# zhouzypaul/fql

Hardware: AMD Instinct MI355X
Metric: FQL gradient-steps/s (batch=256) (higher is better)
Workload: dtype f32

## Files before the change

fql_amd/csrc/fql_engine.hip:

```cpp
#include "../../include/fql_amd.h"
#include "fql_kernels.h"
#include "fql_conv.h"
#include "fql_chain.h"
#include "fql_aux.h"
#include "fql_ifql.h"
#include "fql_rebrac.h"
#include "fql_sac.h"
#include "fql_bc.h"
#include "fql_iql.h"
#include "fql_iqld.h"
#include "fql_cfgrl.h"
#include <hip/hip_ext.h>
#include "fql_aql.h"

#include <algorithm>
#include <cmath>
#include <cstdarg>
#include <cstdio>
#include <cstdlib>
#include <cstring>
#include <map>
#include <memory>
#include <random>
#include <string>
// ... 198 lines not shown
    std::vector<WgradTask> h_wgrad;
    std::vector<LnBwdTask> h_ln;
    std::vector<MiscTask> h_misc;
    bool ka = false;
    std::vector<int> waits;
    bool record_after = false;
    hipEvent_t ev = nullptr;
};

inline bool ka_tasks_env() {
    const char* e = getenv("FQL_KERNARG_TASKS");
    return !e || atoi(e) != 0;
}
inline bool fused_tail_env() {
    const char* e = getenv("FQL_FUSED_TAIL");
    return !e || atoi(e) != 0;
}
inline bool aql_acquire_env() {
    const char* e = getenv("FQL_AQL_ACQUIRE");
    return e && atoi(e) != 0;
}
inline bool l1_independent_kernel(const void* fn) {
#define FQL_L1_CHAIN(HH)                                                                                                                             \
    (const void*)fql_chain_kernel<HH, 0>, (const void*)fql_chain_kernel<HH, 1>, (const void*)fql_chain_kernel<HH, 2>, (const void*)fql_chain_kernel<HH, 3>, \
    (const void*)fql_chain_multi_kernel<HH, 0>, (const void*)fql_chain_multi_kernel<HH, 1>, (const void*)fql_chain_multi_kernel<HH, 2>,             \
    (const void*)fql_chain_multi_kernel<HH, 3>, (const void*)fql_chain_split_kernel<HH, 0>, (const void*)fql_chain_split_kernel<HH, 1>,             \
    (const void*)fql_chain_split_kernel<HH, 2>
    static const void* const table[] = {
        (const void*)fql_prep_kernel, (const void*)fql_prep_multi_kernel,
        (const void*)fql_gemm16_kernel<false>, (const void*)fql_gemm16_kernel<true>,
// ... 312 lines not shown
    float* in_noise[5] = {nullptr, nullptr, nullptr, nullptr, nullptr};
    int64_t* in_idx = nullptr;
    float *X_os = nullptr, *X_bc = nullptr, *X_eu = nullptr, *X_c1 = nullptr, *X_c2 = nullptr, *X_ct = nullptr;
    float *vel = nullptr, *w_rew = nullptr, *w_mask = nullptr, *w_act = nullptr, *tgt = nullptr;
    float *X_e0 = nullptr, *C0 = nullptr, *Abuf[2] = {nullptr, nullptr}, *Vpart = nullptr;
    bool fused_euler = false;
    bool use_chain = false;
    int fill_lane_full = 1;
    std::vector<float*> wf_bc;
    float *wf_w0 = nullptr, *wf_w4 = nullptr;
    WfragTask* d_wfrag = nullptr;
    std::vector<WfragTask> h_wfrag;
    int wfrag_n = 0, wfrag_grid = 0;
    const bool ka_tasks = ka_tasks_env();
    const bool fused_tail = fused_tail_env();
    unsigned* d_ticket = nullptr;
    std::vector<void*> chain_allocs;
    bool split_build = false;
    bool wide_tiles = false;
    bool split_ok = false;
    int vp_tiles = 0;
    int num_cus = 0;
    PassBuf p_os, p_os_bwd, p_bc, p_eu, p_c1[2], p_c2[2], p_ct[2];
    Program prog_fwdbwd, prog_opt, prog_loss;
    Program prog_opt_split;
    Program prog_full;
    int mod_chunk0[3] = {0, 0, 0}, mod_chunkn[3] = {0, 0, 0};
    Program prog_split;
    hipGraphExec_t split_exec[4] = {nullptr, nullptr, nullptr, nullptr};
    hipGraph_t split_graph[4] = {nullptr, nullptr, nullptr, nullptr};
// ... 450 lines not shown
        HIP_CHECK(hipMemcpy(P, h.data(), n_total * sizeof(float), hipMemcpyHostToDevice));
    }

    PassBuf make_pass(std::vector<void*>& owner, int net, int M, float* x0, bool bwd, bool input_grad) {
        const Net& n = nets[net];
        PassBuf p;
        p.net = net; p.M = M; p.x0 = x0;
        const int L = n.nl() - 1;
        for (int l = 0; l < L; ++l) {
            const int H = n.layers[l].out_p;
            p.g.push_back(dalloc(owner, (size_t)M * H));
            p.z.push_back(dalloc(owner, (size_t)M * H));
            if (n.layers[l].ln) {
                p.xn.push_back(dalloc(owner, (size_t)M * H));
                p.stats.push_back(dalloc(owner, (size_t)M * 2));
                p.lnpart.push_back(dalloc(owner, (size_t)M * ((2 * ((H + 31) / 32) + 3) & ~3)));
            } else {
                p.xn.push_back(p.g.back());
                p.stats.push_back(nullptr);
                p.lnpart.push_back(nullptr);
            }
        }
        p.out = dalloc(owner, (size_t)M * n.layers[L].out_p);
        if (bwd) {
            for (int l = 0; l <= L; ++l) p.dz.push_back(dalloc(owner, (size_t)M * n.layers[l].out_p));
            for (int l = 0; l < L; ++l) p.dy.push_back(n.layers[l].ln ? dalloc(owner, (size_t)M * n.layers[l].out_p) : nullptr);
            if (input_grad) p.dx0 = dalloc(owner, (size_t)M * n.in_p());
        }
        return p;
    }

// ... 253 lines not shown

    void push(Program& pr, Op& op) {
        op.lane = emit_lane;
        pr.ops.push_back(op);
    }
    Op& emit(Program& pr, OpType type, const Bound& k, std::vector<const void*> reads, std::vector<const void*> writes) {
        Op op{};
        op.type = type;
        op.k = k;
        op.reads = std::move(reads);
        op.writes = std::move(writes);
        push(pr, op);
        return pr.ops.back();
    }

    void emit_forward(Program& pr, const PassBuf& p, bool save, int final_flags = 0, float* aux = nullptr,
                      float* aux2 = nullptr, float f0 = 0.f, float f1 = 0.f, int first_layer = 0) {
        const Net& n = nets[p.net];
        const int L = n.nl() - 1;
        for (int l = first_layer; l <= L; ++l) {
            const Layer& ly = n.layers[l];
            Op op{};
            op.type = OP_GEMM;
            GemmTask& t = op.gemm;
            const bool a_ln = l > 0 && n.layers[l - 1].ln;
            t.A = (l == 0) ? p.x0 : p.g[l - 1];
            t.lda = ly.in_p;
            t.B = P + ly.w; t.ldb = ly.out_p;
            t.bias = P + ly.b;
            t.M = p.M; t.N = ly.out_p; t.K = ly.in_p;
            t.ldc = ly.out_p;
            t.flags = GF_BIAS;
            op.reads = {t.A, t.B};
            if (a_ln) {
                t.flags |= GF_A_LN;
// ... 4 lines not shown
                    t.ln_xout = p.xn[l - 1]; t.ln_stats = p.stats[l - 1];
                    op.writes.push_back(t.ln_xout);
                    op.writes.push_back(t.ln_stats);
                }
            }
            if (l < L) {
                t.C = p.g[l];
                t.flags |= GF_GELU;
                if (save) { t.flags |= GF_SAVE_Z; t.Zout = p.z[l]; op.writes.push_back(t.Zout); }
                op.writes.push_back(t.C);
                const bool prev64 = l > 0 && want64(p.M, n.layers[l - 1].out_p, n.layers[l - 1].in_p, GF_BIAS | GF_GELU);
                if (want64(t.M, t.N, t.K, t.flags) && (!a_ln || prev64)) {
                    op.type = OP_GEMM64;
                    if (a_ln) { t.aux2 = p.lnpart[l - 1]; t.i0 = t.K / 32; op.reads.push_back(t.aux2); }
                    if (ly.ln) { t.flags |= GF_LN_PART; t.aux = p.lnpart[l]; t.i1 = t.N / 32; op.writes.push_back(t.aux); }
                }
            } else {
                t.C = p.out;
                t.flags |= final_flags;
                if (final_flags & GF_EULER) {
                    t.aux = aux; t.aux2 = aux2;
                    t.i0 = n.in_p(); t.i1 = cfg.obs_dim; t.i2 = cfg.act_dim;
                    t.f0 = f0; t.f1 = f1;
                    op.reads.push_back(aux);
                    op.writes.push_back(aux);
                    if (aux2) op.writes.push_back(aux2);
                } else {
                    op.writes.push_back(t.C);
                    if (final_flags & GF_OS_SCATTER) {
                        t.aux = aux; t.aux2 = aux2;
                        t.i0 = nets[NET_C0].in_p(); t.i1 = cfg.obs_dim; t.i2 = cfg.act_dim;
                        op.writes.push_back(aux);
                        op.writes.push_back(aux2);
                    }
                }
            }
            push(pr, op);
        }
    }

    void emit_euler_fused(Program& pr) {
        const Net& n = nets[NET_BC];
        const int nh = n.nl() - 1, fs = cfg.flow_steps;
        const int od = cfg.obs_dim, ad = cfg.act_dim, ap = pad16(ad), inp_b = n.in_p();
        const Layer& l0 = n.layers[0];
        {
            Op op{};
            op.type = OP_GEMM;
            GemmTask& t = op.gemm;
            t.A = X_e0; t.lda = l0.in_p; t.B = P + l0.w; t.ldb = l0.out_p; t.bias = P + l0.b; t.C = C0; t.ldc = l0.out_p;
            t.M = B; t.N = l0.out_p; t.K = l0.in_p; t.flags = GF_BIAS;
            op.reads = {X_e0, t.B};
            op.writes = {C0};
// ... 146 lines not shown
    }
    void emit_wfrag(Program& pr) {
        if (!use_chain) return;
        const Net& n = nets[NET_BC];
        Op op{};
        op.type = OP_WFRAG;
        op.k = tl_last(bind(fql_wfrag_kernel, wfrag_grid, d_wfrag, wfrag_n, -1));
        for (const Layer& L : n.layers) op.reads.push_back(P + L.w);
        for (float* w : wf_bc) op.writes.push_back(w);
        op.writes.push_back(wf_w0);
        op.writes.push_back(wf_w4);
        push(pr, op);
    }

    void emit_backward(Program& pr, const PassBuf& p, int row_off, int M, bool param_grads, bool input_grad,
                       const void* align_with = nullptr) {
        size_t first_op = pr.ops.size();
        const Net& n = nets[p.net];
        const int L = n.nl() - 1;
        auto rows = [&](float* base, int ld) { return base + (size_t)row_off * ld; };
        auto ln_bwd = [&](int l, const void* first_read) {
            const Layer& prev = n.layers[l - 1];
            Op lo{};
            lo.type = OP_LNBWD;
            LnBwdTask& q = lo.ln;
            q.Z = rows(p.z[l - 1], prev.out_p);
            q.Gv = rows(p.g[l - 1], prev.out_p);
            q.stats = p.stats[l - 1] + (size_t)row_off * 2;
            q.gamma = P + prev.g;
            q.dZ = p.dz[l - 1];
            q.dgamma = param_grads ? G + prev.g : nullptr;
// ... 19 lines not shown
                w.db = G + ly.b;
                w.M = M; w.Kin = ly.in_p; w.N = ly.out_p;
                op.reads = {xin_id, dz};
                op.writes = {w.dW, w.db};
                const int keep = emit_lane;
                if (emit_lane == 0 && !split_build && !lane0_64) emit_lane = 1;
                if (defer_wgrads) { op.lane = emit_lane; defer_wgrads->push_back(op); }
                else push(pr, op);
                emit_lane = keep;
            }
            if (l == 0 && !input_grad) break;
            if (l == L && l > 0 && ly.out == 1 && n.layers[l - 1].ln) {
                Op lo = ln_bwd(l, dz);
                LnBwdTask& q = lo.ln;
                q.dq = dz; q.ldq = ly.out_p; q.wq = P + ly.w; q.ldw = ly.out_p;
                push(pr, lo);
                continue;
            }
            Op op{};
            op.type = OP_GEMM;
            GemmTask& t = op.gemm;
            t.A = dz; t.lda = ly.out_p;
            t.B = P + ly.w; t.ldb = ly.out_p;
            t.M = M; t.N = ly.in_p; t.K = ly.out_p;
            t.ldc = ly.in_p;
            t.flags = GF_TRANS_B;
            op.reads = {dz, t.B};
            if (l == 0) {
                t.C = p.dx0;
                op.writes = {t.C};
// ... 349 lines not shown
            GemmTask t = o->gemm;
            t.wk = (t.N <= 16) ? 4 : 2;
            t.tmt = 1;
            t.ntn = (t.N / 16 + (4 / t.wk) - 1) / (4 / t.wk);
            t.tile0 = tile;
            tile += (t.M / 16) * t.ntn;
            L.h_gemm.push_back(t);
        }
        L.table = upload(owner, L.h_gemm.data(), L.h_gemm.size() * sizeof(GemmTask));
        L.grid = tile;
        bind_gemm16(L);
        return L;
    }

    static double op_macs(const Op& o) {
        if (o.type == OP_GEMM || o.type == OP_GEMM64 || o.type == OP_HEAD_DGRAD) return (double)o.gemm.M * o.gemm.N * o.gemm.K;
        if (o.type == OP_DGRAD0) return (double)o.gemm.M * 16.0 * o.gemm.K;
        if (o.type == OP_WGRAD) return (double)o.wgrad.M * o.wgrad.Kin * o.wgrad.N;
        if (o.type == OP_CHAIN) return o.macs;
        if (o.type == OP_CONV || o.type == OP_CONV_U8) return (double)o.conv.N * o.conv.H * o.conv.W * 9.0 * (o.conv.transposed ? o.conv.Ci : o.conv.Ci_real) * o.conv.Co;
        if (o.type == OP_CONV_WGRAD) return (double)o.cw.N * o.cw.H * o.cw.W * 9.0 * o.cw.Ci_real * o.cw.Co;
        return 0.0;
    }
    static void cross_lane_waits(Program& pr) {
        std::vector<int> need(pr.launches.size() * FQL_LANES, -1);
        for (const Op& o : pr.ops) {
            if (o.launch < 0) continue;
            for (int d : o.deps) {
                const int dl = pr.ops[d].launch;
                const int ol = pr.launches[dl].lane;
                int& nd = need[o.launch * FQL_LANES + ol];
// ... 330 lines not shown
        if (!split_build) fill_lane_full = fill_lane;
        wide_tiles = lanes3;
        place("os", 1, true);
        emit_forward(pr, p_os, with_grads, GF_OS_SCATTER, X_ct, X_c2);
        {
            Op op{};
            op.type = OP_POSTOS;
            op.postos = PostOsArgs{p_os.out, w_act, X_ct, X_c2, st, B, od, ad, inp_c, ap};
            op.reads = {p_os.out, w_act};
            op.writes = {I_MSE};
            push(pr, op);
        }
        place("c1f", fill_lane, true);
        for (int e = 0; e < 2; ++e) emit_forward(pr, p_c1[e], with_grads);
        place("ct", lanes3 ? 1 : fill_lane, true);
        for (int e = 0; e < 2; ++e) emit_forward(pr, p_ct[e], false);
        place("c1", fill_lane, true);
        {
            Op op{};
            op.type = OP_LOSS_CRITIC;
            op.lc = LossCriticArgs{p_c1[0].out, p_c1[1].out, p_ct[0].out, p_ct[1].out, w_rew, w_mask,
                                   with_grads ? p_c1[0].dz.back() : nullptr, with_grads ? p_c1[1].dz.back() : nullptr,
                                   st, B, cfg.q_agg, with_grads ? 1 : 0, cfg.discount};
            op.reads = {p_c1[0].out, p_c1[1].out, p_ct[0].out, p_ct[1].out, w_rew, w_mask};
            op.writes = {I_CR};
            if (with_grads) { op.writes.push_back(p_c1[0].dz.back()); op.writes.push_back(p_c1[1].dz.back()); }
            push(pr, op);
        }
        std::vector<Op> late_ops;
        if (!lanes3 && with_grads) defer_wgrads = &late_ops;
        if (with_grads)
            for (int e = 0; e < 2; ++e) emit_backward(pr, p_c1[e], 0, B, true, visual);
        const bool enc_align = !split_build;
        if (with_grads && visual && !enc_align) {
            place("enc", 1, true);
            emit_encoder_backward(pr, eb_c, 0, B, p_c1[0].dx0, p_c1[1].dx0, nets[NET_C0].in_p());
        }
        {
            place("bcf", lanes3 ? 1 : fill_lane, true);
// ... 4 lines not shown
                op.type = OP_LOSS_BC;
                op.lb = LossBcArgs{p_bc.out, vel, with_grads ? p_bc.dz.back() : nullptr, st, B, ad, ap, with_grads ? 1 : 0};
                op.reads = {p_bc.out, vel};
                op.writes = {I_BC};
                if (with_grads) op.writes.push_back(p_bc.dz.back());
                push(pr, op);
            }
            defer_wgrads = nullptr;
            if (with_grads) emit_backward(pr, p_bc, 0, B, true, visual);
            if (with_grads && visual && !enc_align) {
                place("enc", 1, true);
                emit_encoder_backward(pr, eb_bc, 0, B, p_bc.dx0, nullptr, nets[NET_BC].in_p());
            }
        }
        place("c2", 1, true);
        for (int e = 0; e < 2; ++e) emit_forward(pr, p_c2[e], with_grads);
        {
            Op op{};
            op.type = OP_LOSS_Q;
            const bool dyn_dq = with_grads && cfg.normalize_q_loss;
            op.lq = LossQArgs{p_c2[0].out, p_c2[1].out, dyn_dq ? p_c2[0].dz.back() : nullptr,
                              dyn_dq ? p_c2[1].dz.back() : nullptr, st, B, cfg.normalize_q_loss, dyn_dq ? 1 : 0};
            op.reads = {p_c2[0].out, p_c2[1].out};
            op.writes = {I_Q};
            if (dyn_dq) { op.writes.push_back(p_c2[0].dz.back()); op.writes.push_back(p_c2[1].dz.back()); }
            push(pr, op);
        }
        defer_wgrads = nullptr;
        if (with_grads) {
            for (int e = 0; e < 2; ++e) emit_backward(pr, p_c2[e], 0, B, false, true, !lanes3 ? I_CR : nullptr);
        }
        for (Op& w : late_ops) {
            w.reads.push_back(p_c2[0].dx0); w.reads.push_back(p_c2[1].dx0);
            emit_lane = w.lane;
            push(pr, w);
        }
        place("eu", 0, false);
        const int fs = cfg.flow_steps;
        euler_finish_fused = with_grads && !cfg.actor_layer_norm && fused_euler && use_chain && fs > 1 && vp_tiles <= 32;
        if (fused_euler && use_chain) emit_euler_chain(pr);
        else if (fused_euler) emit_euler_fused(pr);
        else
        for (int s = 0; s < fs; ++s)
            emit_forward(pr, p_eu, false, GF_EULER | (s == fs - 1 ? GF_EULER_LAST : 0), X_eu, tgt, 1.0f / (float)fs,
                         (float)(s + 1) / (float)fs);
// ... 3370 lines not shown
```

fql_amd/csrc/fql_kernels.h:

```cpp
#pragma once
#include <hip/hip_runtime.h>
#include <stdint.h>

typedef float f32x4 __attribute__((ext_vector_type(4)));

#define FQL_GAS __attribute__((address_space(1)))
__device__ __forceinline__ float ldg(const float* p) { return *(const FQL_GAS float*)p; }
__device__ __forceinline__ f32x4 ldg4(const float* p) { return *(const FQL_GAS f32x4*)p; }
typedef unsigned u32x4 __attribute__((ext_vector_type(4)));
__device__ __forceinline__ __amdgpu_buffer_rsrc_t ldx_rsrc(const void* base) {
    const uint64_t b = (uint64_t)base;
    const uint64_t u = ((uint64_t)(unsigned)__builtin_amdgcn_readfirstlane((int)(b >> 32)) << 32) | (unsigned)__builtin_amdgcn_readfirstlane((int)b);
    return __builtin_amdgcn_make_buffer_rsrc((void*)u, 0, 0x7FFFFFFF, 0x00020000);
}
__device__ __forceinline__ float ldx(const float* p) { return __hip_atomic_load((const FQL_GAS float*)p, __ATOMIC_RELAXED, __HIP_MEMORY_SCOPE_AGENT); }
__device__ __forceinline__ u32x4 ldx4u(const unsigned* base, unsigned i, unsigned s = 0) {
    return __builtin_amdgcn_raw_buffer_load_b128(ldx_rsrc(base), (int)(i * 4u), __builtin_amdgcn_readfirstlane((int)(s * 4u)), 16);
}
typedef float f32x2 __attribute__((ext_vector_type(2)));
typedef unsigned u32x2 __attribute__((ext_vector_type(2)));
__device__ __forceinline__ f32x2 ldx2(const float* base, unsigned i, unsigned s = 0) {
    return __builtin_bit_cast(f32x2, __builtin_amdgcn_raw_buffer_load_b64(ldx_rsrc(base), (int)(i * 4u), __builtin_amdgcn_readfirstlane((int)(s * 4u)), 16));
}
__device__ __forceinline__ f32x4 ldx4(const float* base, unsigned i, unsigned s = 0) { return __builtin_bit_cast(f32x4, ldx4u((const unsigned*)base, i, s)); }
// ... 82 lines not shown
    GF_LN_WRITE = 1 << 5,
    GF_GELUGRAD = 1 << 6,
    GF_EULER = 1 << 7,
    GF_EULER_LAST = 1 << 8,
    GF_CLIP_OUT = 1 << 9,
    GF_A_EULER0 = 1 << 11,
    GF_HEAD_PART = 1 << 12,
    GF_OS_SCATTER = 1 << 13,
    GF_A_LOSSACT = 1 << 17,
    GF_A_EULFIN = 1 << 15,
    GF_RELUGRAD = 1 << 14,
    GF_LN_PART = 1 << 10,
    GF_C_FRAGT = 1 << 16,
    GF_C_FRAG = 1 << 18,
    GF_EULER_BARE = 1 << 19,
};

struct GemmTask {
    const float* A;
    const float* B;
    const float* bias;
    float* C;
    float* Zout;
    const float* Zprev;
    const float* ln_g;
    const float* ln_b;
    float* ln_xout;
    float* ln_stats;
    float* aux;
    float* aux2;
// ... 683 lines not shown
        f32x4 pv[NR][4];
#pragma unroll
        for (int i = 0; i < NR; ++i) {
            const unsigned po = (unsigned)((row_first + 16 * i) * rs);
#pragma unroll
            for (int t = 0; t < 4; ++t) pv[i][t] = ldx4(partials, po + 4 * min(base + t, nf4 - 1));
        }
#pragma unroll
        for (int i = 0; i < NR; ++i)
#pragma unroll
            for (int t = 0; t < 4; ++t) {
                if (2 * (base + t) < ntin) { sum[i] += pv[i][t][0]; sumsq[i] += pv[i][t][1]; }
                if (2 * (base + t) + 1 < ntin) { sum[i] += pv[i][t][2]; sumsq[i] += pv[i][t][3]; }
            }
    }
}

template <bool transb, int RI>
__device__ __forceinline__ void gemm64_body(const GemmTask& T, float* lds) {
    constexpr int TM = 32 * RI;
    float* As = lds;
    float* Bs = lds + 2 * TM * G64_S;
    float* part = Bs + 2 * 64 * G64_S;
    const int local = (int)blockIdx.x - T.tile0;
    const int tm = sdiv(local, frcp(T.ntn)), tn = local - tm * T.ntn;
    const int row0 = tm * TM, n0 = tn * 64;
    const int K = T.K;
    const int tid = threadIdx.x, wave = tid >> 6, lane = tid & 63;
    const int wr = wave >> 1, wc = wave & 1;
    const int c = lane & 15, q = lane >> 4;
// ... 248 lines not shown
                }
                if (ln_wr) stg4(T.ln_xout + (size_t)(row0 + sr + 16 * i) * T.lda + k, ra[i]);
            }
        }
#pragma unroll
        for (int i = 0; i < 2; ++i) *reinterpret_cast<f32x4*>(a + (sr + 16 * i) * G64_S + 4 * sc4) = ra[i];
#pragma unroll
        for (int i = 0; i < NB; ++i) *reinterpret_cast<f32x4*>(b + (br0 + brs * i) * BS + 4 * bc4) = rb[i];
    };
    f32x4 acc[NJ][2];
#pragma unroll
    for (int j = 0; j < NJ; ++j) acc[j][0] = acc[j][1] = f32x4{0.f, 0.f, 0.f, 0.f};
    f32x4 bias[NJ];
#pragma unroll
    for (int j = 0; j < NJ; ++j) bias[j] = (flags & GF_BIAS) ? ldg4(T.bias + n0 + (wc * NJ + j) * 16 + 4 * q) : f32x4{0.f, 0.f, 0.f, 0.f};

    auto compute = [&](int buf) {
        const float* a = As + buf * 32 * G64_S + (16 * wr + c) * G64_S + 4 * q;
        const float* b = Bs + buf * BROWS * BS;
        f32x4 fa[2], fb[2][NJ];
        auto read_frags = [&](int slot, int g) {
            fa[slot] = *reinterpret_cast<const f32x4*>(a + 16 * g);
#pragma unroll
            for (int j = 0; j < NJ; ++j) {
                const int col = (wc * NJ + j) * 16 + c;
                if (transb) fb[slot][j] = *reinterpret_cast<const f32x4*>(b + col * BS + 16 * g + 4 * q);
                else {
#pragma unroll
                    for (int s4 = 0; s4 < 4; ++s4) fb[slot][j][s4] = b[(16 * g + 4 * q + s4) * BS + col];
                }
// ... 16 lines not shown
    TSTAMP();
    for (int ch = 0; ch < nchunks; ch += 2) {
        compute(0);
        if (ch + 1 < nchunks) store_chunk(ra1, rb1, lg1, lb1, 64 * (ch + 1), 1);
        __syncthreads();
        if (ch + 3 < nchunks) load_chunk(ra1, rb1, lg1, lb1, 64 * (ch + 3));
        if (ch + 1 < nchunks) {
            compute(1);
            if (ch + 2 < nchunks) store_chunk(ra0, rb0, lg0, lb0, 64 * (ch + 2), 0);
            __syncthreads();
            if (ch + 4 < nchunks) load_chunk(ra0, rb0, lg0, lb0, 64 * (ch + 4));
        }
    }
    TSTAMP();

    float s1 = 0.f, s2 = 0.f;
    {
        const int row = row0 + 16 * wr + c;
#pragma unroll
        for (int j = 0; j < NJ; ++j) {
            const int n = n0 + (wc * NJ + j) * 16 + 4 * q;
            const size_t o = (size_t)row * T.ldc + n;
            f32x4 v = acc[j][0] + acc[j][1] + bias[j];
            if (flags & GF_SAVE_Z) {
                f32x4 dgv;
#pragma unroll
                for (int r = 0; r < 4; ++r) { float gg, dg; gelu_both(v[r], gg, dg); dgv[r] = dg; v[r] = (flags & GF_GELU) ? gg : v[r]; }
                stg4(T.Zout + o, dgv);
            } else if (flags & GF_GELU) {
#pragma unroll
                for (int r = 0; r < 4; ++r) v[r] = gelu_f(v[r]);
            }
            if (flags & GF_GELUGRAD) v *= ldx4(T.Zprev + (size_t)row0 * T.ldc, (unsigned)((16 * wr + c) * T.ldc + n));
            if (flags & GF_RELUGRAD) {
                const f32x4 zp = ldx4(T.Zprev + (size_t)row0 * T.ldc, (unsigned)((16 * wr + c) * T.ldc + n));
#pragma unroll
                for (int r = 0; r < 4; ++r) v[r] = (zp[r] > 0.f) ? v[r] : 0.f;
            }
            stg4(T.C + o, v);
#pragma unroll
            for (int r = 0; r < 4; ++r) { s1 += v[r]; s2 += v[r] * v[r]; }
        }
    }
    if (flags & GF_LN_PART) {
        s1 += __shfl_xor(s1, 16); s2 += __shfl_xor(s2, 16);
        s1 += __shfl_xor(s1, 32); s2 += __shfl_xor(s2, 32);
        if (q == 0) {
            const int rl = 16 * wr + c;
            part[(wc * 32 + rl) * 2] = s1;
            part[(wc * 32 + rl) * 2 + 1] = s2;
        }
        __syncthreads();
        const int rs = (2 * T.i1 + 3) & ~3;
        if (NJ == 2) {
            if (tid < 64) {
                const int half = tid >> 5, rl = tid & 31;
                float* pp = T.aux + (size_t)(row0 + rl) * rs + 2 * (2 * tn + half);
                stg(pp, part[(half * 32 + rl) * 2]);
                stg(pp + 1, part[(half * 32 + rl) * 2 + 1]);
            }
        } else if (tid < 32) {
            float* pp = T.aux + (size_t)(row0 + tid) * rs + 2 * tn;
            stg(pp, part[tid * 2] + part[(32 + tid) * 2]);
            stg(pp + 1, part[tid * 2 + 1] + part[(32 + tid) * 2 + 1]);
        }
    }
#ifdef FQL_STAMPS
    TSTAMP();
    if (tid == 0 && T.stamps64) {
// ... 99 lines not shown
            else {
                const int k = br0 + brs * i;
                const int key = (NJ == 2) ? ((k >> 1) & 3) : ((k >> 2) & 1);
                w = k * RW + 8 * ((bc4 >> 2) ^ key) + 2 * (bc4 & 3);
            }
            *reinterpret_cast<u32x2*>(bh + w) = hi;
            *reinterpret_cast<u32x2*>(bh + BPL + w) = lo;
        }
    };
    f32x4 acc[NJ][2];
#pragma unroll
    for (int j = 0; j < NJ; ++j) acc[j][0] = acc[j][1] = f32x4{0.f, 0.f, 0.f, 0.f};
    f32x4 bias[NJ];
#pragma unroll
    for (int j = 0; j < NJ; ++j) bias[j] = (flags & GF_BIAS) ? ldg4(T.bias + n0 + (wc * NJ + j) * 16 + 4 * q) : f32x4{0.f, 0.f, 0.f, 0.f};

    const int a_row = (16 * wr + c) * 32, sw = (c >> 1) & 7;
    const int qq = c >> 2, p = c & 3;
    const int tr_row = 4 * q + qq;
    const int tr_key = (NJ == 2) ? ((tr_row >> 1) & 3) : ((tr_row >> 2) & 1);
    auto compute = [&](int buf) {
        const unsigned* ah = As + buf * 2 * APL;
        const unsigned* bh = Bs + buf * 2 * BPL;
#pragma unroll
        for (int kp = 0; kp < 2; ++kp) {
            const int slot = 4 * ((4 * kp + q) ^ sw);
            const u32x4 fah = *reinterpret_cast<const u32x4*>(ah + a_row + slot);
            const u32x4 fal = *reinterpret_cast<const u32x4*>(ah + APL + a_row + slot);
            u32x4 fbh[NJ], fbl[NJ];
#pragma unroll
// ... 24 lines not shown
    SSTAMP();
    for (int ch = 0; ch < nchunks; ch += 2) {
        compute(0);
        if (ch + 1 < nchunks) store_chunk(ra1, rb1, lg1, lb1, 64 * (ch + 1), 1);
        __syncthreads();
        if (ch + 3 < nchunks) load_chunk(ra1, rb1, lg1, lb1, 64 * (ch + 3));
        if (ch + 1 < nchunks) {
            compute(1);
            if (ch + 2 < nchunks) store_chunk(ra0, rb0, lg0, lb0, 64 * (ch + 2), 0);
            __syncthreads();
            if (ch + 4 < nchunks) load_chunk(ra0, rb0, lg0, lb0, 64 * (ch + 4));
        }
    }

    SSTAMP();
    float s1 = 0.f, s2 = 0.f;
    {
        const int row = row0 + 16 * wr + c;
#pragma unroll
        for (int j = 0; j < NJ; ++j) {
            const int n = n0 + (wc * NJ + j) * 16 + 4 * q;
            const size_t o = (size_t)row * T.ldc + n;
            f32x4 v = acc[j][0] + acc[j][1] + bias[j];
            if (flags & GF_SAVE_Z) {
                f32x4 dgv;
#pragma unroll
                for (int r = 0; r < 4; ++r) { float gg, dg; gelu_both(v[r], gg, dg); dgv[r] = dg; v[r] = (flags & GF_GELU) ? gg : v[r]; }
                stg4(T.Zout + o, dgv);
            } else if (flags & GF_GELU) {
#pragma unroll
                for (int r = 0; r < 4; ++r) v[r] = gelu_f(v[r]);
            }
            if (flags & GF_GELUGRAD) v *= ldx4(T.Zprev + (size_t)row0 * T.ldc, (unsigned)((16 * wr + c) * T.ldc + n));
            if (flags & GF_RELUGRAD) {
                const f32x4 zp = ldx4(T.Zprev + (size_t)row0 * T.ldc, (unsigned)((16 * wr + c) * T.ldc + n));
#pragma unroll
                for (int r = 0; r < 4; ++r) v[r] = (zp[r] > 0.f) ? v[r] : 0.f;
            }
            stg4(T.C + o, v);
#pragma unroll
            for (int r = 0; r < 4; ++r) { s1 += v[r]; s2 += v[r] * v[r]; }
        }
    }
    if (flags & GF_LN_PART) {
        s1 += __shfl_xor(s1, 16); s2 += __shfl_xor(s2, 16);
        s1 += __shfl_xor(s1, 32); s2 += __shfl_xor(s2, 32);
        if (q == 0) {
            const int rl = 16 * wr + c;
            part[(wc * 32 + rl) * 2] = s1;
            part[(wc * 32 + rl) * 2 + 1] = s2;
        }
        __syncthreads();
        const int rs = (2 * T.i1 + 3) & ~3;
        if (NJ == 2) {
            if (tid < 64) {
                const int half = tid >> 5, rl = tid & 31;
                float* pp = T.aux + (size_t)(row0 + rl) * rs + 2 * (2 * tn + half);
                stg(pp, part[(half * 32 + rl) * 2]);
                stg(pp + 1, part[(half * 32 + rl) * 2 + 1]);
            }
        } else if (tid < 32) {
            float* pp = T.aux + (size_t)(row0 + tid) * rs + 2 * tn;
            stg(pp, part[tid * 2] + part[(32 + tid) * 2]);
            stg(pp + 1, part[tid * 2 + 1] + part[(32 + tid) * 2 + 1]);
        }
    }
#ifdef FQL_STAMPS
    SSTAMP();
    if (tid == 0 && T.stamps64) {
// ... 171 lines not shown
        if (s + 8 < steps) {
            if (s + 16 < steps) load(a0, b0, s + 16);
            mma(a1, b1, s + 8);
        }
    }
    wgrad_finish<1>(T, lds, acc, bs, tk, k0, n0, ntv, true);
}

template <bool SYN>
__device__ __forceinline__ void lnbwd_body(const LnBwdTask& T, int bid, float (*red)[16][16]) {
    const int local = bid - T.tile0;
    const int wave = threadIdx.x >> 6, lane = threadIdx.x & 63;
    if (local < T.ntiles_rows) {
        const int row = local * 4 + wave;
        if (row >= T.M) return;
        const float mean = ldx(T.stats + 2 * row), rstd = ldx(T.stats + 2 * row + 1);
        const unsigned ro = (unsigned)(row * T.ld);
        const float dqr = SYN ? ldx(T.dq + (size_t)row * T.ldq) : 0.f;
        f32x4 zz[4], dd[4], gm[4], gq[4];
#pragma unroll
        for (int i = 0; i < 4; ++i) {
            const int k4 = 4 * (lane + 64 * i);
            if (k4 < T.H) {
                zz[i] = ldx4(T.Z, ro + k4);
                gq[i] = ldx4(T.Gv, ro + k4);
                gm[i] = ldg4(T.gamma + k4);
                if (SYN) {
#pragma unroll
                    for (int e = 0; e < 4; ++e) dd[i][e] = dqr * ldg(T.wq + (size_t)(k4 + e) * T.ldw);
                } else dd[i] = ldx4(T.dY, ro + k4);
            } else zz[i] = gq[i] = gm[i] = dd[i] = f32x4{0.f, 0.f, 0.f, 0.f};
        }
        f32x4 d[4], xh[4];
        float s1 = 0.f, s2 = 0.f;
#pragma unroll
        for (int i = 0; i < 4; ++i)
#pragma unroll
            for (int e = 0; e < 4; ++e) {
                const int k = 4 * (lane + 64 * i) + e;
                xh[i][e] = (gq[i][e] - mean) * rstd;
                d[i][e] = dd[i][e] * gm[i][e];
                if (k < T.width) { s1 += d[i][e]; s2 += d[i][e] * xh[i][e]; }
            }
#pragma unroll
        for (int o = 1; o < 64; o <<= 1) {
            s1 += __shfl_xor(s1, o);
            s2 += __shfl_xor(s2, o);
// ... 167 lines not shown
    for (int o = 1; o < 64; o <<= 1) v += __shfl_xor(v, o);
    __syncthreads();
    if ((threadIdx.x & 63) == 0) sh[threadIdx.x >> 6] = v;
    __syncthreads();
    return sh[0] + sh[1] + sh[2] + sh[3];
}
__device__ __forceinline__ float block_max(float v, float* sh) {
#pragma unroll
    for (int o = 1; o < 64; o <<= 1) v = fmaxf(v, __shfl_xor(v, o));
    __syncthreads();
    if ((threadIdx.x & 63) == 0) sh[threadIdx.x >> 6] = v;
    __syncthreads();
    return fmaxf(fmaxf(sh[0], sh[1]), fmaxf(sh[2], sh[3]));
}

struct PostOsArgs {
    const float* A_os;
    const float* w_act;
    float *X_ct, *X_c2;
    DevState* st;
    int B, od, ad, inp_c, ap;
};
__device__ __forceinline__ void fql_post_onestep_body(const PostOsArgs& P, float* sh) {
    float se = 0.f;
    const int n = P.B * P.ad;
    for (int e = threadIdx.x; e < n; e += FQL_THREADS) {
        const int b = sdiv(e, frcp(P.ad)), a = e - b * P.ad;
        const float d = clip1(ldx(P.A_os + (size_t)(2 * P.B + b) * P.ap + a)) - ldx(P.w_act + (size_t)b * P.ap + a);
        se += d * d;
    }
    const float tot = block_sum(se, sh);
    if (threadIdx.x == 0) P.st->info[9] = tot / (float)n;
}

struct LossCriticArgs {
    const float *q1a, *q1b, *tqa, *tqb;
    const float *w_rew, *w_mask;
    float *dq1a, *dq1b;
    DevState* st;
    int B, q_agg, want_grad;
    float discount;
};
__device__ __forceinline__ void fql_loss_critic_body(const LossCriticArgs& P, float* sh) {
    float sl = 0.f, sq = 0.f, mx = -INFINITY, mn = INFINITY;
    const float gs = 1.0f / (float)P.B;
    for (int b = threadIdx.x; b < P.B; b += FQL_THREADS) {
        const float ta = ldx(P.tqa + (size_t)b * 16), tb = ldx(P.tqb + (size_t)b * 16);
        const float nq = P.q_agg ? fminf(ta, tb) : 0.5f * (ta + tb);
        const float y = ldx(P.w_rew + b) + P.discount * ldx(P.w_mask + b) * nq;
        const float qa = ldx(P.q1a + (size_t)b * 16), qb = ldx(P.q1b + (size_t)b * 16);
        const float da = qa - y, db = qb - y;
        sl += da * da + db * db;
        sq += qa + qb;
        mx = fmaxf(mx, fmaxf(qa, qb));
        mn = fminf(mn, fminf(qa, qb));
        if (P.want_grad) {
            P.dq1a[(size_t)b * 16] = da * gs;
            P.dq1b[(size_t)b * 16] = db * gs;
        }
    }
    const float tl = block_sum(sl, sh), tq = block_sum(sq, sh);
    const float tmx = block_max(mx, sh), tmn = -block_max(-mn, sh);
    if (threadIdx.x == 0) {
        const float inv = 1.0f / (2.0f * (float)P.B);
        P.st->info[0] = tl * inv;
        P.st->info[1] = tq * inv;
        P.st->info[2] = tmx;
        P.st->info[3] = tmn;
    }
}

struct LossQArgs {
    const float *q2a, *q2b;
    float *dq2a, *dq2b;
    DevState* st;
    int B, normalize, want_grad;
};
__device__ __forceinline__ void fql_loss_q_body(const LossQArgs& P, float* sh) {
    float s = 0.f, sa = 0.f;
    for (int b = threadIdx.x; b < P.B; b += FQL_THREADS) {
        const float q = 0.5f * (ldx(P.q2a + (size_t)b * 16) + ldx(P.q2b + (size_t)b * 16));
        s += q; sa += fabsf(q);
    }
    const float ts = block_sum(s, sh), tsa = block_sum(sa, sh);
    const float qmean = ts / (float)P.B;
    const float lam = P.normalize ? 1.0f / (tsa / (float)P.B) : 1.0f;
    if (P.want_grad) {
        const float g = -lam / (2.0f * (float)P.B);
        for (int b = threadIdx.x; b < P.B; b += FQL_THREADS) {
            P.dq2a[(size_t)b * 16] = g;
            P.dq2b[(size_t)b * 16] = g;
        }
    }
    if (threadIdx.x == 0) {
        P.st->info[7] = lam * (-qmean);
        P.st->info[8] = qmean;
// ... 50 lines not shown
    }
    const float t = block_sum(s, sh);
    if (threadIdx.x == 0) {
        const float distill = t / (float)n;
        P.st->info[6] = distill;
        P.st->info[4] = ldx(&P.st->info[5]) + P.alpha * distill + ldx(&P.st->info[7]);
    }
}

__global__ __launch_bounds__(FQL_THREADS) void fql_loss_actor_kernel(LossActorArgs P) { __shared__ float sh[4]; fql_loss_actor_body(P, sh); }
__global__ __launch_bounds__(FQL_THREADS) void fql_loss_actor_multi_kernel(const LossActorArgs* __restrict__ args) { __shared__ float sh[4]; const LossActorArgs P = args[blockIdx.y]; fql_loss_actor_body(P, sh); }

enum : int { MISC_POSTOS = 0, MISC_LOSS_CRITIC, MISC_LOSS_Q, MISC_LOSS_BC };
struct MiscTask {
    int kind;
    union {
        PostOsArgs po;
        LossCriticArgs lc;
        LossQArgs lq;
        LossBcArgs lb;
    };
};

struct AdamChunk { int off, len, leaf; };
struct FinalizeArgs {
    DevState* st;
    const AdamChunk* chunks;
    const float* partials;
    const int* leaf_range;
    int n_chunks, nleaves, do_grad_stats;
// ... 270 lines not shown
    tl_enter(tl);
    side_body<false, true>(gt, ngt, wt, nwt, lt, nlt, tile_w, tile_l, mt, tile_m);
    tl_exit(tl);
}
__global__ __launch_bounds__(FQL_THREADS, 2) void fql_side_big_kernel(
    const GemmTask* __restrict__ gt, int ngt, const WgradTask* __restrict__ wt, int nwt, const LnBwdTask* __restrict__ lt, int nlt, int tile_w, int tile_l,
    const MiscTask* __restrict__ mt, int tile_m, int tl) {
    tl_enter(tl);
    side_body<true>(gt, ngt, wt, nwt, lt, nlt, tile_w, tile_l, mt, tile_m);
    tl_exit(tl);
}

#define FQL_KA_GEMM 8
#define FQL_KA_WGRAD 16
#define FQL_KA_LN 6
#define FQL_KA_MISC 4
struct SideFront {
    int tile_w, tile_l, tile_m, tl;
    int g0[FQL_KA_GEMM - 1];
    int w0[FQL_KA_WGRAD - 1];
    int l0[FQL_KA_LN - 1];
    int pad;
};
struct SideArgs {
    SideFront f;
    GemmTask g[FQL_KA_GEMM];
    WgradTask w[FQL_KA_WGRAD];
    LnBwdTask l[FQL_KA_LN];
    MiscTask m[FQL_KA_MISC];
};
static_assert(sizeof(SideFront) == 128, "the front is two 16-dword loads");
static_assert(sizeof(SideArgs) <= FQL_KA_LIMIT, "SideArgs and the hidden block must fit the 4 KB of a launch's arguments");
template <bool BIG, bool SPLIT = false>
__device__ __forceinline__ void side_ka_body(const SideFront& F) {
    extern __shared__ __attribute__((aligned(16))) float lds[];
    const int b = blockIdx.x;
    if (b < F.tile_w) {
        const GemmTask T = ka_load<GemmTask>(ka_base() + offsetof(SideArgs, g) + (size_t)find_front(F.g0, b) * sizeof(GemmTask));
        gemm_tile_dispatch<BIG, SPLIT>(T, lds);
    } else if (b < F.tile_l) {
        const int bid = b - F.tile_w;
        const WgradTask T = ka_load<WgradTask>(ka_base() + offsetof(SideArgs, w) + (size_t)find_front(F.w0, bid) * sizeof(WgradTask));
        if (SPLIT) wgrad_split_body(T, bid, lds);
        else wgrad_body(T, bid, lds);
    } else if (b < F.tile_m) {
        const int bid = b - F.tile_l;
// ... 33 lines not shown
```

Baseline: 3059.

## Fold critic Q-head GEMM into last hidden layer's LayerNorm partial sums

For critic and target-critic forwards, the scalar Q head after the final LayerNorm layer is no longer run as its own GEMM. The previous layer's epilogue now also accumulates a dot product of the pre-norm activations with gamma times head weights, and the loss kernels rebuild Q from the mean, variance and that sum. The backward LN pass reads the same partials instead of stats. This drops a small GEMM launch or task and the write and read of the head output, at the cost of extra epilogue work, a wider partial buffer, per-loss weight reductions, and a smaller kernel-argument misc slot count.

```diff
diff --git a/fql_amd/csrc/fql_engine.hip b/fql_amd/csrc/fql_engine.hip
--- a/fql_amd/csrc/fql_engine.hip
+++ b/fql_amd/csrc/fql_engine.hip
@@ -236,6 +236,10 @@
 }
 inline bool fused_tail_env() {
     const char* e = getenv("FQL_FUSED_TAIL");
+    return !e || atoi(e) != 0;
+}
+inline bool qhead_fold_env() {
+    const char* e = getenv("FQL_QHEAD_FOLD");
     return !e || atoi(e) != 0;
 }
 inline bool aql_acquire_env() {
@@ -578,6 +582,7 @@
     int wfrag_n = 0, wfrag_grid = 0;
     const bool ka_tasks = ka_tasks_env();
     const bool fused_tail = fused_tail_env();
+    const bool qhead_fold = qhead_fold_env();
     unsigned* d_ticket = nullptr;
     std::vector<void*> chain_allocs;
     bool split_build = false;
@@ -1058,7 +1063,7 @@
             if (n.layers[l].ln) {
                 p.xn.push_back(dalloc(owner, (size_t)M * H));
                 p.stats.push_back(dalloc(owner, (size_t)M * 2));
-                p.lnpart.push_back(dalloc(owner, (size_t)M * ((2 * ((H + 31) / 32) + 3) & ~3)));
+                p.lnpart.push_back(dalloc(owner, (size_t)M * 4 * ((H + 31) / 32)));
             } else {
                 p.xn.push_back(p.g.back());
                 p.stats.push_back(nullptr);
@@ -1342,11 +1347,13 @@
         return pr.ops.back();
     }
 
-    void emit_forward(Program& pr, const PassBuf& p, bool save, int final_flags = 0, float* aux = nullptr,
-                      float* aux2 = nullptr, float f0 = 0.f, float f1 = 0.f, int first_layer = 0) {
+    bool emit_forward(Program& pr, const PassBuf& p, bool save, int final_flags = 0, float* aux = nullptr,
+                      float* aux2 = nullptr, float f0 = 0.f, float f1 = 0.f, int first_layer = 0, bool qfold = false) {
         const Net& n = nets[p.net];
         const int L = n.nl() - 1;
+        bool folded = false;
         for (int l = first_layer; l <= L; ++l) {
+            if (l == L && folded) break;
             const Layer& ly = n.layers[l];
             Op op{};
             op.type = OP_GEMM;
@@ -1381,6 +1388,17 @@
                     op.type = OP_GEMM64;
                     if (a_ln) { t.aux2 = p.lnpart[l - 1]; t.i0 = t.K / 32; op.reads.push_back(t.aux2); }
                     if (ly.ln) { t.flags |= GF_LN_PART; t.aux = p.lnpart[l]; t.i1 = t.N / 32; op.writes.push_back(t.aux); }
+                    const Layer& head = n.layers[L];
+                    if (qfold && l == L - 1 && ly.ln && head.out == 1 && final_flags == 0 && side_ri(t) == 1) {
+                        if (ly.be != ly.g + ly.out_p || head.w != ly.be + ly.out_p || head.out_p != 16 || head.b != head.w + (size_t)ly.out_p * 16)
+                            invalid("internal: a folded head's parameters are not contiguous in the arena");
+                        t.flags |= GF_QH_PART;
+                        t.ew = P + ly.g; t.ew4 = P + head.w; t.e_ntp = head.out_p; t.i2 = ly.out;
+                        op.reads.push_back(t.ew);
+                        op.reads.push_back(t.ew4);
+                        op.macs = (double)t.M * head.out_p * head.in_p;
+                        folded = true;
+                    }
                 }
             } else {
                 t.C = p.out;
@@ -1404,6 +1422,13 @@
             }
             push(pr, op);
         }
+        return folded;
+    }
+    struct QhArgs { const float *part, *gam; int hp, width; std::vector<const void*> reads; };
+    QhArgs qh_args(const PassBuf& p) const {
+        const Net& n = nets[p.net];
+        const Layer &ly = n.layers[n.nl() - 2], &head = n.layers[n.nl() - 1];
+        return QhArgs{p.lnpart[n.nl() - 2], P + ly.g, ly.out_p, ly.out, {p.lnpart[n.nl() - 2], P + ly.w, P + ly.g, P + head.w}};
     }
 
     void emit_euler_fused(Program& pr) {
@@ -1580,7 +1605,8 @@
     }
 
     void emit_backward(Program& pr, const PassBuf& p, int row_off, int M, bool param_grads, bool input_grad,
-                       const void* align_with = nullptr) {
+                       const void* align_with = nullptr, bool qfold = false) {
+        if (qfold && (param_grads || row_off != 0)) invalid("internal: a folded head's backward pass carries no parameter gradients");
         size_t first_op = pr.ops.size();
         const Net& n = nets[p.net];
         const int L = n.nl() - 1;
@@ -1630,6 +1656,10 @@
                 Op lo = ln_bwd(l, dz);
                 LnBwdTask& q = lo.ln;
                 q.dq = dz; q.ldq = ly.out_p; q.wq = P + ly.w; q.ldw = ly.out_p;
+                if (qfold) {
+                    q.dY = p.lnpart[l - 1]; q.stats = nullptr;
+                    std::replace(lo.reads.begin(), lo.reads.end(), (const void*)p.stats[l - 1], (const void*)p.lnpart[l - 1]);
+                }
                 push(pr, lo);
                 continue;
             }
@@ -2009,7 +2039,7 @@
     }
 
     static double op_macs(const Op& o) {
-        if (o.type == OP_GEMM || o.type == OP_GEMM64 || o.type == OP_HEAD_DGRAD) return (double)o.gemm.M * o.gemm.N * o.gemm.K;
+        if (o.type == OP_GEMM || o.type == OP_GEMM64 || o.type == OP_HEAD_DGRAD) return (double)o.gemm.M * o.gemm.N * o.gemm.K + o.macs;
         if (o.type == OP_DGRAD0) return (double)o.gemm.M * 16.0 * o.gemm.K;
         if (o.type == OP_WGRAD) return (double)o.wgrad.M * o.wgrad.Kin * o.wgrad.N;
         if (o.type == OP_CHAIN) return o.macs;
@@ -2370,15 +2400,23 @@
         place("c1f", fill_lane, true);
         for (int e = 0; e < 2; ++e) emit_forward(pr, p_c1[e], with_grads);
         place("ct", lanes3 ? 1 : fill_lane, true);
-        for (int e = 0; e < 2; ++e) emit_forward(pr, p_ct[e], false);
+        const bool qf = qhead_fold && lanes3;
+        bool f_ct[2], f_c2[2];
+        for (int e = 0; e < 2; ++e) f_ct[e] = emit_forward(pr, p_ct[e], false, 0, nullptr, nullptr, 0.f, 0.f, 0, qf);
+        if (f_ct[0] != f_ct[1]) invalid("internal: the target critic members differ in shape");
         place("c1", fill_lane, true);
         {
             Op op{};
             op.type = OP_LOSS_CRITIC;
             op.lc = LossCriticArgs{p_c1[0].out, p_c1[1].out, p_ct[0].out, p_ct[1].out, w_rew, w_mask,
                                    with_grads ? p_c1[0].dz.back() : nullptr, with_grads ? p_c1[1].dz.back() : nullptr,
-                                   st, B, cfg.q_agg, with_grads ? 1 : 0, cfg.discount};
-            op.reads = {p_c1[0].out, p_c1[1].out, p_ct[0].out, p_ct[1].out, w_rew, w_mask};
+                                   st, B, cfg.q_agg, with_grads ? 1 : 0, cfg.discount, nullptr, nullptr, 0, 0};
+            op.reads = {p_c1[0].out, p_c1[1].out, w_rew, w_mask};
+            if (f_ct[0]) {
+                const QhArgs a = qh_args(p_ct[0]), b = qh_args(p_ct[1]);
+                op.lc.tqa = a.part; op.lc.tqb = b.part; op.lc.tga = a.gam; op.lc.tgb = b.gam; op.lc.hp = a.hp; op.lc.width = a.width;
+                for (const QhArgs* q : {&a, &b}) op.reads.insert(op.reads.end(), q->reads.begin(), q->reads.end());
+            } else { op.reads.push_back(p_ct[0].out); op.reads.push_back(p_ct[1].out); }
             op.writes = {I_CR};
             if (with_grads) { op.writes.push_back(p_c1[0].dz.back()); op.writes.push_back(p_c1[1].dz.back()); }
             push(pr, op);
@@ -2413,21 +2451,31 @@
             }
         }
         place("c2", 1, true);
-        for (int e = 0; e < 2; ++e) emit_forward(pr, p_c2[e], with_grads);
+        for (int e = 0; e < 2; ++e) f_c2[e] = emit_forward(pr, p_c2[e], with_grads, 0, nullptr, nullptr, 0.f, 0.f, 0, qf);
+        if (f_c2[0] != f_c2[1]) invalid("internal: the critic members differ in shape");
         {
             Op op{};
             op.type = OP_LOSS_Q;
             const bool dyn_dq = with_grads && cfg.normalize_q_loss;
             op.lq = LossQArgs{p_c2[0].out, p_c2[1].out, dyn_dq ? p_c2[0].dz.back() : nullptr,
-                              dyn_dq ? p_c2[1].dz.back() : nullptr, st, B, cfg.normalize_q_loss, dyn_dq ? 1 : 0};
+                              dyn_dq ? p_c2[1].dz.back() : nullptr, st, B, cfg.normalize_q_loss, dyn_dq ? 1 : 0, nullptr, nullptr, 0, 0};
             op.reads = {p_c2[0].out, p_c2[1].out};
+            if (f_c2[0]) {
+                const QhArgs a = qh_args(p_c2[0]), b = qh_args(p_c2[1]);
+                op.lq.q2a = a.part; op.lq.q2b = b.part; op.lq.ga = a.gam; op.lq.gb = b.gam; op.lq.hp = a.hp; op.lq.width = a.width;
+                op.reads.clear();
+                for (const QhArgs* q : {&a, &b}) op.reads.insert(op.reads.end(), q->reads.begin(), q->reads.end());
+            }
             op.writes = {I_Q};
             if (dyn_dq) { op.writes.push_back(p_c2[0].dz.back()); op.writes.push_back(p_c2[1].dz.back()); }
+            const int keep = emit_lane;
+            if (f_c2[0] && !dyn_dq) emit_lane = fill_lane;
             push(pr, op);
+            emit_lane = keep;
         }
         defer_wgrads = nullptr;
         if (with_grads) {
-            for (int e = 0; e < 2; ++e) emit_backward(pr, p_c2[e], 0, B, false, true, !lanes3 ? I_CR : nullptr);
+            for (int e = 0; e < 2; ++e) emit_backward(pr, p_c2[e], 0, B, false, true, !lanes3 ? I_CR : nullptr, f_c2[e]);
         }
         for (Op& w : late_ops) {
             w.reads.push_back(p_c2[0].dx0); w.reads.push_back(p_c2[1].dx0);
diff --git a/fql_amd/csrc/fql_kernels.h b/fql_amd/csrc/fql_kernels.h
--- a/fql_amd/csrc/fql_kernels.h
+++ b/fql_amd/csrc/fql_kernels.h
@@ -120,6 +120,7 @@
     GF_C_FRAGT = 1 << 16,
     GF_C_FRAG = 1 << 18,
     GF_EULER_BARE = 1 << 19,
+    GF_QH_PART = 1 << 20,
 };
 
 struct GemmTask {
@@ -833,6 +834,40 @@
                 if (2 * (base + t) + 1 < ntin) { sum[i] += pv[i][t][2]; sumsq[i] += pv[i][t][3]; }
             }
     }
+}
+
+__device__ __forceinline__ f32x4 qh_weights(const GemmTask& T, int n) {
+    const f32x4 g = ldg4(T.ew + n);
+    f32x4 u;
+#pragma unroll
+    for (int r = 0; r < 4; ++r) u[r] = (n + r < T.i2) ? g[r] * ldg(T.ew4 + (size_t)(n + r) * T.e_ntp) : 0.f;
+    return u;
+}
+__device__ __forceinline__ float qh_fold(const float* __restrict__ part, int row, int nt, int width, float sgw, float sbw, float hb, float& mean, float& rstd) {
+    float s1 = 0.f, s2 = 0.f, s3 = 0.f;
+    const unsigned ro = (unsigned)(row * nt) * 4u;
+    for (int base = 0; base < nt; base += 8) {
+        f32x4 pv[8];
+#pragma unroll
+        for (int t = 0; t < 8; ++t) pv[t] = ldx4(part, ro + 4u * (unsigned)min(base + t, nt - 1));
+#pragma unroll
+        for (int t = 0; t < 8; ++t)
+            if (base + t < nt) { s1 += pv[t][0]; s2 += pv[t][1]; s3 += pv[t][2]; }
+    }
+    const float inv = 1.0f / (float)width;
+    mean = s1 * inv;
+    const float var = fmaxf(0.0f, s2 * inv - mean * mean);
+    rstd = 1.0f / sqrtf(var + 1e-6f);
+    return rstd * (s3 - mean * sgw) + sbw + hb;
+}
+__device__ __forceinline__ void qh_fold_wave(const float* __restrict__ part, int row, int nt, int width, int lane, float& mean, float& rstd) {
+    const f32x4 r = ldx4(part, (unsigned)(row * nt + min(lane, nt - 1)) * 4u);
+    float s1 = 0.f, s2 = 0.f;
+    for (int p = 0; p < nt; ++p) { s1 += __shfl(r[0], p); s2 += __shfl(r[1], p); }
+    const float inv = 1.0f / (float)width;
+    mean = s1 * inv;
+    const float var = fmaxf(0.0f, s2 * inv - mean * mean);
+    rstd = 1.0f / sqrtf(var + 1e-6f);
 }
 
 template <bool transb, int RI>
@@ -1111,6 +1146,9 @@
     f32x4 bias[NJ];
 #pragma unroll
     for (int j = 0; j < NJ; ++j) bias[j] = (flags & GF_BIAS) ? ldg4(T.bias + n0 + (wc * NJ + j) * 16 + 4 * q) : f32x4{0.f, 0.f, 0.f, 0.f};
+    f32x4 qu[NJ];
+#pragma unroll
+    for (int j = 0; j < NJ; ++j) qu[j] = (flags & GF_QH_PART) ? qh_weights(T, n0 + (wc * NJ + j) * 16 + 4 * q) : f32x4{0.f, 0.f, 0.f, 0.f};
 
     auto compute = [&](int buf) {
         const float* a = As + buf * 32 * G64_S + (16 * wr + c) * G64_S + 4 * q;
@@ -1157,7 +1195,8 @@
     }
     TSTAMP();
 
-    float s1 = 0.f, s2 = 0.f;
+    float s1 = 0.f, s2 = 0.f, s3 = 0.f;
+    float* part3 = lds;
     {
         const int row = row0 + 16 * wr + c;
 #pragma unroll
@@ -1182,20 +1221,33 @@
             }
             stg4(T.C + o, v);
 #pragma unroll
-            for (int r = 0; r < 4; ++r) { s1 += v[r]; s2 += v[r] * v[r]; }
+            for (int r = 0; r < 4; ++r) { s1 += v[r]; s2 += v[r] * v[r]; s3 = fmaf(v[r], qu[j][r], s3); }
         }
     }
     if (flags & GF_LN_PART) {
+        const bool qh = (flags & GF_QH_PART) != 0;
         s1 += __shfl_xor(s1, 16); s2 += __shfl_xor(s2, 16);
         s1 += __shfl_xor(s1, 32); s2 += __shfl_xor(s2, 32);
+        if (qh) { s3 += __shfl_xor(s3, 16); s3 += __shfl_xor(s3, 32); }
         if (q == 0) {
             const int rl = 16 * wr + c;
             part[(wc * 32 + rl) * 2] = s1;
             part[(wc * 32 + rl) * 2 + 1] = s2;
+            if (qh) part3[wc * 32 + rl] = s3;
         }
         __syncthreads();
         const int rs = (2 * T.i1 + 3) & ~3;
-        if (NJ == 2) {
+        if (qh) {
+            if (NJ == 2) {
+                if (tid < 64) {
+                    const int half = tid >> 5, rl = tid & 31, pi = half * 32 + rl;
+                    stg4(T.aux + ((size_t)(row0 + rl) * T.i1 + 2 * tn + half) * 4, f32x4{part[pi * 2], part[pi * 2 + 1], part3[pi], 0.f});
+                }
+            } else if (tid < 32) {
+                stg4(T.aux + ((size_t)(row0 + tid) * T.i1 + tn) * 4,
+                     f32x4{part[tid * 2] + part[(32 + tid) * 2], part[tid * 2 + 1] + part[(32 + tid) * 2 + 1], part3[tid] + part3[32 + tid], 0.f});
+            }
+        } else if (NJ == 2) {
             if (tid < 64) {
                 const int half = tid >> 5, rl = tid & 31;
                 float* pp = T.aux + (size_t)(row0 + rl) * rs + 2 * (2 * tn + half);
@@ -1325,6 +1377,9 @@
     f32x4 bias[NJ];
 #pragma unroll
     for (int j = 0; j < NJ; ++j) bias[j] = (flags & GF_BIAS) ? ldg4(T.bias + n0 + (wc * NJ + j) * 16 + 4 * q) : f32x4{0.f, 0.f, 0.f, 0.f};
+    f32x4 qu[NJ];
+#pragma unroll
+    for (int j = 0; j < NJ; ++j) qu[j] = (flags & GF_QH_PART) ? qh_weights(T, n0 + (wc * NJ + j) * 16 + 4 * q) : f32x4{0.f, 0.f, 0.f, 0.f};
 
     const int a_row = (16 * wr + c) * 32, sw = (c >> 1) & 7;
     const int qq = c >> 2, p = c & 3;
@@ -1379,7 +1434,8 @@
     }
 
     SSTAMP();
-    float s1 = 0.f, s2 = 0.f;
+    float s1 = 0.f, s2 = 0.f, s3 = 0.f;
+    float* part3 = lds_f;
     {
         const int row = row0 + 16 * wr + c;
 #pragma unroll
@@ -1404,20 +1460,33 @@
             }
             stg4(T.C + o, v);
 #pragma unroll
-            for (int r = 0; r < 4; ++r) { s1 += v[r]; s2 += v[r] * v[r]; }
+            for (int r = 0; r < 4; ++r) { s1 += v[r]; s2 += v[r] * v[r]; s3 = fmaf(v[r], qu[j][r], s3); }
         }
     }
     if (flags & GF_LN_PART) {
+        const bool qh = (flags & GF_QH_PART) != 0;
         s1 += __shfl_xor(s1, 16); s2 += __shfl_xor(s2, 16);
         s1 += __shfl_xor(s1, 32); s2 += __shfl_xor(s2, 32);
+        if (qh) { s3 += __shfl_xor(s3, 16); s3 += __shfl_xor(s3, 32); }
         if (q == 0) {
             const int rl = 16 * wr + c;
             part[(wc * 32 + rl) * 2] = s1;
             part[(wc * 32 + rl) * 2 + 1] = s2;
+            if (qh) part3[wc * 32 + rl] = s3;
         }
         __syncthreads();
         const int rs = (2 * T.i1 + 3) & ~3;
-        if (NJ == 2) {
+        if (qh) {
+            if (NJ == 2) {
+                if (tid < 64) {
+                    const int half = tid >> 5, rl = tid & 31, pi = half * 32 + rl;
+                    stg4(T.aux + ((size_t)(row0 + rl) * T.i1 + 2 * tn + half) * 4, f32x4{part[pi * 2], part[pi * 2 + 1], part3[pi], 0.f});
+                }
+            } else if (tid < 32) {
+                stg4(T.aux + ((size_t)(row0 + tid) * T.i1 + tn) * 4,
+                     f32x4{part[tid * 2] + part[(32 + tid) * 2], part[tid * 2 + 1] + part[(32 + tid) * 2 + 1], part3[tid] + part3[32 + tid], 0.f});
+            }
+        } else if (NJ == 2) {
             if (tid < 64) {
                 const int half = tid >> 5, rl = tid & 31;
                 float* pp = T.aux + (size_t)(row0 + rl) * rs + 2 * (2 * tn + half);
@@ -1619,7 +1688,9 @@
     if (local < T.ntiles_rows) {
         const int row = local * 4 + wave;
         if (row >= T.M) return;
-        const float mean = ldx(T.stats + 2 * row), rstd = ldx(T.stats + 2 * row + 1);
+        const bool fold = SYN && T.dY != nullptr;
+        float mean = 0.f, rstd = 1.f;
+        if (!fold) { mean = ldx(T.stats + 2 * row); rstd = ldx(T.stats + 2 * row + 1); }
         const unsigned ro = (unsigned)(row * T.ld);
         const float dqr = SYN ? ldx(T.dq + (size_t)row * T.ldq) : 0.f;
         f32x4 zz[4], dd[4], gm[4], gq[4];
@@ -1636,6 +1707,7 @@
                 } else dd[i] = ldx4(T.dY, ro + k4);
             } else zz[i] = gq[i] = gm[i] = dd[i] = f32x4{0.f, 0.f, 0.f, 0.f};
         }
+        if (fold) qh_fold_wave(T.dY, row, T.H >> 5, T.width, lane, mean, rstd);
         f32x4 d[4], xh[4];
         float s1 = 0.f, s2 = 0.f;
 #pragma unroll
@@ -1833,6 +1905,22 @@
     return fmaxf(fmaxf(sh[0], sh[1]), fmaxf(sh[2], sh[3]));
 }
 
+struct QhNet { float sgw, sbw, hb; };
+__device__ __forceinline__ QhNet qh_sums(const float* gam, int hp, int width, float* sh) {
+    const float *bet = gam + hp, *w = gam + 2 * hp;
+    float sg = 0.f, sb = 0.f;
+    for (int n = threadIdx.x; n < width; n += FQL_THREADS) {
+        const float wn = ldg(w + (size_t)n * 16);
+        sg = fmaf(ldg(gam + n), wn, sg);
+        sb = fmaf(ldg(bet + n), wn, sb);
+    }
+    QhNet r;
+    r.sgw = block_sum(sg, sh);
+    r.sbw = block_sum(sb, sh);
+    r.hb = ldg(w + (size_t)hp * 16);
+    return r;
+}
+
 struct PostOsArgs {
     const float* A_os;
     const float* w_act;
@@ -1859,12 +1947,21 @@
     DevState* st;
     int B, q_agg, want_grad;
     float discount;
+    const float *tga, *tgb;
+    int hp, width;
 };
 __device__ __forceinline__ void fql_loss_critic_body(const LossCriticArgs& P, float* sh) {
     float sl = 0.f, sq = 0.f, mx = -INFINITY, mn = INFINITY;
     const float gs = 1.0f / (float)P.B;
+    const bool ft = P.tga != nullptr;
+    QhNet na{}, nb{};
+    if (ft) { na = qh_sums(P.tga, P.hp, P.width, sh); nb = qh_sums(P.tgb, P.hp, P.width, sh); }
     for (int b = threadIdx.x; b < P.B; b += FQL_THREADS) {
-        const float ta = ldx(P.tqa + (size_t)b * 16), tb = ldx(P.tqb + (size_t)b * 16);
+        float ta, tb, mean, rstd;
+        if (ft) {
+            ta = qh_fold(P.tqa, b, P.hp >> 5, P.width, na.sgw, na.sbw, na.hb, mean, rstd);
+            tb = qh_fold(P.tqb, b, P.hp >> 5, P.width, nb.sgw, nb.sbw, nb.hb, mean, rstd);
+        } else { ta = ldx(P.tqa + (size_t)b * 16); tb = ldx(P.tqb + (size_t)b * 16); }
         const float nq = P.q_agg ? fminf(ta, tb) : 0.5f * (ta + tb);
         const float y = ldx(P.w_rew + b) + P.discount * ldx(P.w_mask + b) * nq;
         const float qa = ldx(P.q1a + (size_t)b * 16), qb = ldx(P.q1b + (size_t)b * 16);
@@ -1894,11 +1991,21 @@
     float *dq2a, *dq2b;
     DevState* st;
     int B, normalize, want_grad;
+    const float *ga, *gb;
+    int hp, width;
 };
 __device__ __forceinline__ void fql_loss_q_body(const LossQArgs& P, float* sh) {
     float s = 0.f, sa = 0.f;
+    const bool fq = P.ga != nullptr;
+    QhNet na{}, nb{};
+    if (fq) { na = qh_sums(P.ga, P.hp, P.width, sh); nb = qh_sums(P.gb, P.hp, P.width, sh); }
     for (int b = threadIdx.x; b < P.B; b += FQL_THREADS) {
-        const float q = 0.5f * (ldx(P.q2a + (size_t)b * 16) + ldx(P.q2b + (size_t)b * 16));
+        float qa, qb, mean, rstd;
+        if (fq) {
+            qa = qh_fold(P.q2a, b, P.hp >> 5, P.width, na.sgw, na.sbw, na.hb, mean, rstd);
+            qb = qh_fold(P.q2b, b, P.hp >> 5, P.width, nb.sgw, nb.sbw, nb.hb, mean, rstd);
+        } else { qa = ldx(P.q2a + (size_t)b * 16); qb = ldx(P.q2b + (size_t)b * 16); }
+        const float q = 0.5f * (qa + qb);
         s += q; sa += fabsf(q);
     }
     const float ts = block_sum(s, sh), tsa = block_sum(sa, sh);
@@ -1979,6 +2086,7 @@
 enum : int { MISC_POSTOS = 0, MISC_LOSS_CRITIC, MISC_LOSS_Q, MISC_LOSS_BC };
 struct MiscTask {
     int kind;
+    int pad[3];
     union {
         PostOsArgs po;
         LossCriticArgs lc;
@@ -2279,7 +2387,7 @@
 #define FQL_KA_GEMM 8
 #define FQL_KA_WGRAD 16
 #define FQL_KA_LN 6
-#define FQL_KA_MISC 4
+#define FQL_KA_MISC 3
 struct SideFront {
     int tile_w, tile_l, tile_m, tl;
     int g0[FQL_KA_GEMM - 1];
@@ -2295,6 +2403,7 @@
     MiscTask m[FQL_KA_MISC];
 };
 static_assert(sizeof(SideFront) == 128, "the front is two 16-dword loads");
+static_assert(sizeof(MiscTask) == 128, "a loss / metric task is one 32-dword ka_load");
 static_assert(sizeof(SideArgs) <= FQL_KA_LIMIT, "SideArgs and the hidden block must fit the 4 KB of a launch's arguments");
 template <bool BIG, bool SPLIT = false>
 __device__ __forceinline__ void side_ka_body(const SideFront& F) {
```

After: 3037. No clear change (-0.7%).
